# KikeM/romtime

Measured on AMD Instinct MI355X. Metric: snapshot-DoF/s for POD build, higher is better.
Workload: dtype f64

## Files before the change

### include/romtime_hip.h

```cpp
#ifndef ROMTIME_HIP_H
#define ROMTIME_HIP_H

#include <stdint.h>

#ifdef __cplusplus
extern "C" {
#endif

typedef struct rt_ctx rt_ctx;

#define RT_OK 0
#define RT_ERR_ARG (-1)
#define RT_ERR_HIP (-2)
#define RT_ERR_UNSUPPORTED (-3)
#define RT_WARN_ZERO_NORM 1
#define RT_WARN_SINGULAR 2

#define RT_ROW_MAJOR 0
#define RT_COL_MAJOR 1

int rt_version(void);
int rt_ctx_create(rt_ctx** out, int device);
void rt_ctx_destroy(rt_ctx* ctx);
int rt_ctx_set_stream(rt_ctx* ctx, void* hip_stream);
// ... 127 lines not shown
                                      int64_t stride_a, const double* scale, int64_t n_pts, int64_t k, int64_t nt,
                                      int64_t n_traj, int fn, const double* par, const double* out, int64_t* info3);

int rt_interpolation_errors(rt_ctx* ctx, const double* Psi, int64_t ldpsi, const int64_t* idx, int64_t m, const double* F,
                            int64_t ldf, int f_layout, int64_t N, int64_t S, int64_t group, int64_t pin_row, double pin_value,
                            double* err, double* ref);
int rt_interpolation_errors_plan_info(int num_cus, const double* Psi, int64_t ldpsi, const int64_t* idx, int64_t m,
                                      const double* F, int64_t ldf, int f_layout, int64_t N, int64_t S, int64_t group,
                                      int64_t pin_row, double pin_value, const double* err, const double* ref, int64_t* info3);

#define RT_P1_MASS 0
#define RT_P1_STIFFNESS 1
#define RT_P1_CONVECTION 2
#define RT_P1_TRILINEAR 3
#define RT_P1_LOAD 4
#define RT_P1_LOAD_P2 5
int rt_p1_local_assembly(rt_ctx* ctx, int kind, int64_t nx, const int64_t* rows, const int64_t* cols, int64_t m,
                         int64_t n_states, const double* h, const double* coef, int state_mode, const double* state,
                         double* out);

int rt_p1_snapshot_sets(rt_ctx* ctx, int kind, int64_t nx, const int64_t* rows, const int64_t* cols, int64_t m,
                        int64_t n_par, const double* h, const double* coef, int par_mode, const double* par,
                        int64_t n_fun, const double* fun, int zero_first, double beta, double* out);
int rt_p1_snapshot_sets_plan_info(int num_cus, int kind, int64_t nx, const int64_t* rows, const int64_t* cols, int64_t m,
                                  int64_t n_par, const double* h, const double* coef, int par_mode, const double* par,
                                  int64_t n_fun, const double* fun, int zero_first, double beta, const double* out,
                                  int64_t* info2);

typedef struct {
  int64_t nx, n_mu, nt;
  int64_t first_step;
  double dt;
  int bdf2;
  int state_in_w;
  const double* tab;
  const double* u_init;
} rt_fom_desc;
int rt_p1_fom_bdf_sweep(rt_ctx* ctx, const rt_fom_desc* desc, double* U_out, int64_t ld_step, int64_t stride_mu, int* info);
int rt_p1_fom_bdf_sweep_plan_info(int num_cus, const rt_fom_desc* desc, int64_t ld_step, int64_t stride_mu, int64_t* info3);
int rt_p1_fom_bdf_sweep_certified(rt_ctx* ctx, const rt_fom_desc* desc, double* U_out, int64_t ld_step, int64_t stride_mu,
                                  double defect_tol, double* defect, int* info);
int rt_p1_fom_bdf_sweep_certified_plan_info(int num_cus, const rt_fom_desc* desc, int64_t ld_step, int64_t stride_mu,
                                            int64_t* info4);

int rt_trajectory_residuals(rt_ctx* ctx, const rt_fom_desc* desc, const double* B, int64_t ldb, int64_t k, const double* A,
                            int64_t lda, int64_t stride_a, const double* a_init, double* res, double* scale);
int rt_trajectory_residuals_plan_info(int num_cus, const rt_fom_desc* desc, const double* B, int64_t ldb, int64_t k,
                                      const double* A, int64_t lda, int64_t stride_a, const double* a_init, const double* res,
                                      const double* scale, int64_t* info3);

int rt_sym_eig_values(rt_ctx* ctx, const double* G, int64_t n, double* lam, int* status);
int rt_sym_eig_values_part(rt_ctx* ctx, const double* G, int64_t n, int64_t first, int64_t count, double* lam,
                           int* status);
int rt_sym_eig_vectors(rt_ctx* ctx, int64_t n, int64_t k, const double* lam, double* W);

int rt_sym_jacobi_eigh(rt_ctx* ctx, const double* A, int64_t n, double* lam, double* W, int max_sweeps, int* sweeps_done,
                       int* status);

int rt_sym_eig_blocked_plan_info(int64_t n, int64_t block_max, int64_t* p_out, int64_t* widths);
#define RT_EIG_BLOCKED_OK 0
#define RT_EIG_BLOCKED_NOT_REDUCIBLE 1
#define RT_EIG_BLOCKED_SOLVE_FAILED 2
int rt_sym_eig_blocked(rt_ctx* ctx, const double* G, int64_t n, double floor_rel, int64_t k, double* lam, double* W,
                       int64_t* resolved, int64_t* block_ranks, int* status);

int rt_host_jacobi_eigh(double* A, int64_t n, double* W, double* lam, int max_sweeps, int* sweeps_done);

int rt_bench_mfma_f64(rt_ctx* ctx, int iters, double* tflops);
int rt_bench_copy(rt_ctx* ctx, void* dst, const void* src, int64_t bytes, int reps, double* gbps);

#ifdef __cplusplus
}
#endif
#endif
```

### romtime_amd/_lib.py

```python
from __future__ import annotations

import ctypes as C
import os
import threading
import weakref

_HERE = os.path.dirname(os.path.abspath(__file__))
LIB_PATH = os.path.join(_HERE, "lib", "libromtime_hip.so")

ROW_MAJOR, COL_MAJOR = 0, 1
RT_OK = 0
WARN_ZERO_NORM, WARN_SINGULAR = 1, 2
EIG_BLOCKED_OK, EIG_BLOCKED_NOT_REDUCIBLE, EIG_BLOCKED_SOLVE_FAILED = 0, 1, 2

_p = C.c_void_p
_i64 = C.c_int64
_int = C.c_int

SOLVER_DIRECT, SOLVER_GMRES = 0, 1


class GmresOpts(C.Structure):

    _fields_ = [("rtol", C.c_double), ("atol", C.c_double), ("restart", _i64), ("maxiter", _i64)]
# ... 7 lines not shown
    "rt_ctx_synchronize": (_int, [_p]),
    "rt_last_error": (C.c_char_p, [_p]),
    "rt_last_launch_info": (_int, [_p, C.POINTER(_i64)]),
    "rt_ctx_set_profile": (_int, [_p, _int]),
    "rt_ctx_set_option": (_int, [_p, C.c_char_p, _int]),
    "rt_last_gemm_ms": (_int, [_p, C.POINTER(C.c_double)]),
    "rt_last_gram_ms": (_int, [_p, C.POINTER(C.c_double)]),
    "rt_gram_plan_info": (_int, [_int, _i64, _i64, C.POINTER(_int)]),
    "rt_gram_spare_plan_info": (_int, [_int, _i64, _i64, _int, _int, C.POINTER(_int)]),
    "rt_ctx_get_counter": (_int, [_p, C.c_char_p, C.POINTER(_i64)]),
    "rt_stream_create_cu_range": (_int, [_int, _int, _int, C.POINTER(_p)]),
    "rt_stream_destroy": (_int, [_p]),
    "rt_last_sweep_stats": (_int, [_p, C.POINTER(_i64)]),
    "rt_gram": (_int, [_p, _p, _i64, _i64, _i64, _int, _p]),
    "rt_gram_scale": (_int, [_p, _p, _i64, _p, _int, _p]),
    "rt_pod_backproject_weights": (_int, [_p, _p, _i64, _i64, _p, _p, _p]),
    "rt_pod_enqueue": (_int, [_p, _p, _i64, _i64, _i64, _int, _i64, _int, _p, _p, _p, _p, _p, _p, _p]),
    "rt_pod_orth": (_int, [_p, _p, _i64, _i64, _i64, _int, _i64, C.c_double, _int, _p, _i64, C.POINTER(_i64), _p, _p,
                           C.POINTER(_int)]),
    "rt_gemm_tn": (_int, [_p, _p, _i64, _int, _p, _i64, _int, _i64, _i64, _i64, _p, _i64]),
    "rt_gemm_nn": (_int, [_p, _p, _i64, _int, _p, _i64, _i64, _i64, _i64, _p, _i64, _int]),
    "rt_rank_update": (_int, [_p, _p, _i64, _p, _p, _i64, _p, _i64, _i64, _i64, _i64, C.c_double, _p, _i64]),
    "rt_gemm_nn_axpby": (_int, [_p, _p, _i64, _int, _p, _i64, _i64, _i64, _i64, C.c_double, C.c_double, _p, _i64, _int]),
    "rt_transpose": (_int, [_p, _p, _i64, _i64, _i64, _p, _i64]),
    "rt_deim_greedy": (_int, [_p, _p, _i64, _i64, _i64, _int, _p, _p, _p]),
    "rt_csr_spmm": (_int, [_p, _p, _p, _p, _i64, _p, _i64, _i64, _p, _i64]),
    "rt_project_csr": (_int, [_p, _p, _p, _p, _i64, _p, _i64, _i64, _p]),
    "rt_project_csr_batched": (_int, [_p, _p, _p, _p, _i64, _int, _i64, _i64, _p, _i64, _i64, _p]),
    "rt_project_stage_info": (_int, [_p, _p, _p, _i64, C.POINTER(_i64), C.POINTER(_int)]),
    "rt_dense_solve_batched": (_int, [_p, _p, _p, _i64, _i64, _p]),
    "rt_dense_solve_multi": (_int, [_p, _p, _i64, _p, _p, _i64, _p]),
    "rt_tracked_solve_batched": (_int, [_p, _p, _p, _p, _i64, _i64, _int, _p]),
    "rt_gmres_batched": (_int, [_p, _p, _p, _p, _i64, _i64, C.POINTER(GmresOpts), _p, _p]),
    "rt_ctx_set_reduced_solver": (_int, [_p, _int, C.POINTER(GmresOpts)]),
    "rt_rom_bdf_sweep": (_int, [_p, _p, _p]),
    "rt_hrom_bdf_sweep": (_int, [_p, _p, _p]),
    "rt_trajectory_errors": (_int, [_p, _p, _i64, _p, _i64, _i64, _p, _i64, _int, _i64, _i64, _i64, _i64, _i64, _p, _p]),
    "rt_trajectory_integrals": (_int, [_p, _p, _i64, _p, _p, _i64, _i64, _p, _i64, _i64, _i64, _i64, _int, C.POINTER(C.c_double), _p]),
    "rt_trajectory_integrals_plan_info": (_int, [_int, _p, _i64, _p, _p, _i64, _i64, _p, _i64, _i64, _i64, _i64, _int,
                                                 C.POINTER(C.c_double), _p, C.POINTER(_i64)]),
    "rt_interpolation_errors": (_int, [_p, _p, _i64, C.POINTER(_i64), _i64, _p, _i64, _int, _i64, _i64, _i64, _i64, C.c_double, _p, _p]),
    "rt_interpolation_errors_plan_info": (_int, [_int, _p, _i64, C.POINTER(_i64), _i64, _p, _i64, _int, _i64, _i64, _i64, _i64,
                                                 C.c_double, _p, _p, C.POINTER(_i64)]),
    "rt_p1_local_assembly": (_int, [_p, _int, _i64, _p, _p, _i64, _i64, _p, _p, _int, _p, _p]),
    "rt_p1_snapshot_sets": (_int, [_p, _int, _i64, _p, _p, _i64, _i64, _p, _p, _int, _p, _i64, _p, _int, C.c_double, _p]),
    "rt_p1_snapshot_sets_plan_info": (_int, [_int, _int, _i64, _p, _p, _i64, _i64, _p, _p, _int, _p, _i64, _p, _int, C.c_double, _p,
                                             C.POINTER(_i64)]),
    "rt_p1_fom_bdf_sweep": (_int, [_p, _p, _p, _i64, _i64, _p]),
    "rt_p1_fom_bdf_sweep_plan_info": (_int, [_int, _p, _i64, _i64, C.POINTER(_i64)]),
    "rt_p1_fom_bdf_sweep_certified": (_int, [_p, _p, _p, _i64, _i64, C.c_double, _p, _p]),
    "rt_p1_fom_bdf_sweep_certified_plan_info": (_int, [_int, _p, _i64, _i64, C.POINTER(_i64)]),
    "rt_trajectory_residuals": (_int, [_p, _p, _p, _i64, _i64, _p, _i64, _i64, _p, _p, _p]),
    "rt_trajectory_residuals_plan_info": (_int, [_int, _p, _p, _i64, _i64, _p, _i64, _i64, _p, _p, _p, C.POINTER(_i64)]),
    "rt_sym_eig_values": (_int, [_p, _p, _i64, _p, _p]),
    "rt_sym_eig_values_part": (_int, [_p, _p, _i64, _i64, _i64, _p, _p]),
    "rt_sym_eig_vectors": (_int, [_p, _i64, _i64, _p, _p]),
    "rt_sym_eig_blocked_plan_info": (_int, [_i64, _i64, C.POINTER(_i64), C.POINTER(_i64)]),
    "rt_sym_eig_blocked": (_int, [_p, _p, _i64, C.c_double, _i64, _p, _p, C.POINTER(_i64), C.POINTER(_i64), C.POINTER(_int)]),
    "rt_sym_jacobi_eigh": (_int, [_p, _p, _i64, _p, _p, _int, C.POINTER(_int), _p]),
    "rt_host_jacobi_eigh": (_int, [_p, _i64, _p, _p, _int, C.POINTER(_int)]),
    "rt_bench_mfma_f64": (_int, [_p, _int, C.POINTER(C.c_double)]),
    "rt_bench_copy": (_int, [_p, _p, _p, _i64, _int, C.POINTER(C.c_double)]),
}



class SweepDesc(C.Structure):

    _fields_ = [("N", _i64), ("nnz", _i64), ("r", _i64), ("n_mu", _i64), ("nt", _i64), ("dt", C.c_double),
                ("bdf2", _int), ("indptr", _p), ("indices", _p), ("V", _p), ("mass_values", _p), ("n_terms", _i64),
                ("term_values", _p), ("term_coef", _p), ("tril_values", _p), ("n_rhs", _i64), ("rhs_terms", _p),
                ("rhs_coef", _p)]


class HSweepDesc(C.Structure):

    _fields_ = [("r", _i64), ("n_mu", _i64), ("nt", _i64), ("dt", C.c_double), ("bdf2", _int), ("m_mass", _i64),
                ("m_lin", _i64), ("m_nl", _i64), ("m_rhs", _i64), ("Z", _p), ("Zf", _p), ("F_mass", _p), ("F_lin", _p),
                ("F_rhs", _p), ("W", _p), ("C_nl", _p), ("S_nl", _p)]


class FomDesc(C.Structure):

    _fields_ = [("nx", _i64), ("n_mu", _i64), ("nt", _i64), ("first_step", _i64), ("dt", C.c_double), ("bdf2", _int),
                ("state_in_w", _int), ("tab", _p), ("u_init", _p)]


_lib = None
_lock = threading.Lock()


class RomtimeHipError(RuntimeError):
    pass


def load():
    global _lib
    with _lock:
        if _lib is not None:
            return _lib
        if not os.path.exists(LIB_PATH):
            raise RomtimeHipError(
                f"{LIB_PATH} is missing: build it with `python -m romtime_amd.build` "
                "(hipcc --offload-arch=gfx950). romtime_amd has no CPU fallback."
            )
        lib = C.CDLL(LIB_PATH)
# ... 146 lines not shown
```

### romtime_amd/csrc/api.hip

```cpp
#include "common.h"

#include <chrono>
#include <new>

namespace {

int grow(rt_ctx* ctx, void** buf, size_t* have, size_t bytes, void** out) {
  if (bytes > *have) {
    RT_HIP_CHECK(ctx, hipStreamSynchronize(ctx->stream));
    if (*buf) RT_HIP_CHECK(ctx, hipFree(*buf));
    *buf = nullptr;
    *have = 0;
    const size_t want = (bytes + ((size_t)1 << 20) - 1) & ~(((size_t)1 << 20) - 1);
    RT_HIP_CHECK(ctx, hipMalloc(buf, want));
    *have = want;
  }
  *out = *buf;
  return RT_OK;
}

__global__ void gram_scale_kernel(double* __restrict__ G, int n, double* __restrict__ colnorm, int normalize,
                                  int* status_flag) {
  const long idx = (long)blockIdx.x * blockDim.x + threadIdx.x;
  if (idx >= (long)n * n) return;
// ... 103 lines not shown
      s += a;
    }
  }
  if (s == -1.2345) sink[0] = s;
}

__global__ __launch_bounds__(256) void copy_kernel(double4* __restrict__ dst, const double4* __restrict__ src, long n4) {
  const long stride = (long)gridDim.x * blockDim.x;
  for (long i = (long)blockIdx.x * blockDim.x + threadIdx.x; i < n4; i += stride) dst[i] = src[i];
}

}

int rt_scratch(rt_ctx* ctx, size_t bytes, void** out) { return grow(ctx, &ctx->scratch, &ctx->scratch_bytes, bytes, out); }
int rt_scratch2(rt_ctx* ctx, size_t bytes, void** out) {
  ++ctx->scratch2_gen;
  return grow(ctx, &ctx->scratch2, &ctx->scratch2_bytes, bytes, out);
}

int rt_func_lds(rt_ctx* ctx, const void* fn, int bytes) {
  for (const void* f : ctx->lds_done)
    if (f == fn) return RT_OK;
  RT_HIP_CHECK(ctx, hipFuncSetAttribute(fn, hipFuncAttributeMaxDynamicSharedMemorySize, bytes));
  ctx->lds_done.push_back(fn);
  return RT_OK;
}

int rt_profile_begin(rt_ctx* ctx, bool also_gram) {
  if (!ctx->profile) return RT_OK;
  if (!ctx->ev0) {
    RT_HIP_CHECK(ctx, hipEventCreate(&ctx->ev0));
    RT_HIP_CHECK(ctx, hipEventCreate(&ctx->ev1));
  }
  if (also_gram && !ctx->gev0) {
    RT_HIP_CHECK(ctx, hipEventCreate(&ctx->gev0));
    RT_HIP_CHECK(ctx, hipEventCreate(&ctx->gev1));
  }
  RT_HIP_CHECK(ctx, hipEventRecord(ctx->ev0, ctx->stream));
  if (also_gram) RT_HIP_CHECK(ctx, hipEventRecord(ctx->gev0, ctx->stream));
  return RT_OK;
}

int rt_profile_end(rt_ctx* ctx, bool also_gram) {
  if (!ctx->profile) return RT_OK;
  RT_HIP_CHECK(ctx, hipEventRecord(ctx->ev1, ctx->stream));
  if (also_gram) RT_HIP_CHECK(ctx, hipEventRecord(ctx->gev1, ctx->stream));
  ctx->ev_valid = true;
  if (also_gram) ctx->gev_valid = true;
  return RT_OK;
}

extern "C" {

int rt_version(void) { return 440; }

int rt_ctx_create(rt_ctx** out, int device) {
  if (!out) return RT_ERR_ARG;
  *out = nullptr;
  int count = 0;
  if (hipGetDeviceCount(&count) != hipSuccess || device < 0 || device >= count) return RT_ERR_HIP;
  if (hipSetDevice(device) != hipSuccess) return RT_ERR_HIP;
  rt_ctx* ctx = new (std::nothrow) rt_ctx();
  if (!ctx) return RT_ERR_HIP;
  ctx->device = device;
  hipDeviceProp_t prop;
  if (hipGetDeviceProperties(&prop, device) == hipSuccess) ctx->num_cus = ctx->device_cus = prop.multiProcessorCount;
  if (hipMalloc(reinterpret_cast<void**>(&ctx->dev_counters), sizeof(long) * RT_N_COUNTERS) != hipSuccess ||
      hipMemset(ctx->dev_counters, 0, sizeof(long) * RT_N_COUNTERS) != hipSuccess) {
    delete ctx;
    return RT_ERR_HIP;
  }
  *out = ctx;
  return RT_OK;
}

void rt_ctx_destroy(rt_ctx* ctx) {
  if (!ctx) return;
  (void)hipSetDevice(ctx->device);
  (void)hipDeviceSynchronize();
  if (ctx->scratch) (void)hipFree(ctx->scratch);
  if (ctx->scratch2) (void)hipFree(ctx->scratch2);
  if (ctx->dev_counters) (void)hipFree(ctx->dev_counters);
  if (ctx->gram_pace) (void)hipFree(ctx->gram_pace);
  if (ctx->ev0) (void)hipEventDestroy(ctx->ev0);
  if (ctx->ev1) (void)hipEventDestroy(ctx->ev1);
  if (ctx->gev0) (void)hipEventDestroy(ctx->gev0);
  if (ctx->gev1) (void)hipEventDestroy(ctx->gev1);
  delete ctx;
}

int rt_ctx_set_stream(rt_ctx* ctx, void* hip_stream) {
  if (!ctx) return RT_ERR_ARG;
  ctx->stream = static_cast<hipStream_t>(hip_stream);
  return RT_OK;
}

int rt_stream_create_cu_range(int device, int first_cu_per_xcd, int n_cu_per_xcd, void** stream) {
  if (!stream) return RT_ERR_ARG;
  *stream = nullptr;
  hipDeviceProp_t prop;
  if (hipSetDevice(device) != hipSuccess || hipGetDeviceProperties(&prop, device) != hipSuccess) return RT_ERR_HIP;
  const int per_xcd = prop.multiProcessorCount / 8;
  if (first_cu_per_xcd < 0 || n_cu_per_xcd < 1 || first_cu_per_xcd + n_cu_per_xcd > per_xcd) return RT_ERR_ARG;
  const int words = (prop.multiProcessorCount + 31) / 32;
  std::vector<uint32_t> mask((size_t)words, 0u);
  for (int cu = first_cu_per_xcd; cu < first_cu_per_xcd + n_cu_per_xcd; ++cu)
    for (int xcd = 0; xcd < 8; ++xcd) {
      const int bit = cu * 8 + xcd;
      mask[bit >> 5] |= 1u << (bit & 31);
    }
  hipStream_t st = nullptr;
  if (hipExtStreamCreateWithCUMask(&st, (uint32_t)words, mask.data()) != hipSuccess) return RT_ERR_HIP;
  *stream = st;
  return RT_OK;
}

int rt_stream_destroy(void* stream) {
  if (!stream) return RT_ERR_ARG;
  return hipStreamDestroy(static_cast<hipStream_t>(stream)) == hipSuccess ? RT_OK : RT_ERR_HIP;
}

int rt_ctx_synchronize(rt_ctx* ctx) {
  if (!ctx) return RT_ERR_ARG;
  RT_HIP_CHECK(ctx, hipStreamSynchronize(ctx->stream));
  return RT_OK;
}

const char* rt_last_error(rt_ctx* ctx) { return ctx ? ctx->err.c_str() : "null ctx"; }

int rt_last_launch_info(rt_ctx* ctx, int64_t* info3) {
  if (!ctx || !info3) return RT_ERR_ARG;
  info3[0] = ctx->last_grid;
  info3[1] = ctx->last_splits;
  info3[2] = ctx->last_tile;
  return RT_OK;
}

int rt_ctx_set_option(rt_ctx* ctx, const char* name, int value) {
  if (!ctx || !name) return RT_ERR_ARG;
  const std::string key(name);
  if (key == "eig_one_xcd") {
    ctx->eig_one_xcd = value != 0;
    return RT_OK;
  }
  if (key == "eig_xcd") {
    if (value < 0 || value > 7) {
      ctx->err = "rt_ctx_set_option: eig_xcd must be 0 .. 7";
      return RT_ERR_ARG;
    }
    ctx->eig_xcd = value;
    return RT_OK;
  }
  if (key == "gram_pace") {
    ctx->gram_pace_on = value != 0;
    return RT_OK;
  }
  if (key == "pod_blocked") {
    ctx->pod_blocked = value != 0;
    return RT_OK;
  }
  if (key == "sweep_graph") {
    ctx->sweep_graph = value != 0;
    return RT_OK;
  }
  if (key == "cu_limit") {
    if (value < 0 || value > ctx->device_cus || (value % 8) != 0) {
      ctx->err = "rt_ctx_set_option: cu_limit must be a multiple of 8 between 0 and the device's CU count";
      return RT_ERR_ARG;
    }
    ctx->num_cus = value ? value : ctx->device_cus;
    return RT_OK;
  }
  ctx->err = "rt_ctx_set_option: unknown option " + key;
  return RT_ERR_ARG;
}

int rt_ctx_get_counter(rt_ctx* ctx, const char* name, int64_t* value) {
  if (!ctx || !name || !value) return RT_ERR_ARG;
  const std::string key(name);
  static const struct { const char* name; int slot; } table[] = {
      {"eig_timeouts", RT_CNT_EIG_TIMEOUT}, {"eig_general_form", RT_CNT_EIG_GENERAL_FORM},
      {"eig_one_xcd", RT_CNT_EIG_ONE_XCD}, {"gram_off_xcd", RT_CNT_GRAM_OFF_XCD}, {"sweep_newton_iterations", RT_CNT_NS_ITER},
      {"sweep_restarts", RT_CNT_NS_RESTART}, {"sweep_lu_fallbacks", RT_CNT_LU_FALLBACK}, {"sweep_solves", RT_CNT_SOLVES},
      {"sweep_gmres_iterations", RT_CNT_GMRES_ITER}, {"sweep_gmres_unconverged", RT_CNT_GMRES_UNCONVERGED},
      {"eig_wide_form", RT_CNT_EIG_WIDE_FORM}, {"eig_blocked", RT_CNT_EIG_BLOCKED},
      {"eig_blocked_not_reducible", RT_CNT_EIG_BLOCKED_NOT_REDUCIBLE}, {"eig_blocked_rank", RT_CNT_EIG_BLOCKED_RANK}};
  for (const auto& t : table)
    if (key == t.name) {
      long host = 0;
      RT_HIP_CHECK(ctx, hipMemcpyAsync(&host, ctx->dev_counters + t.slot, sizeof(long), hipMemcpyDeviceToHost, ctx->stream));
      RT_HIP_CHECK(ctx, hipStreamSynchronize(ctx->stream));
      *value = host;
      return RT_OK;
    }
  ctx->err = "rt_ctx_get_counter: unknown counter " + key;
  return RT_ERR_ARG;
}

int rt_last_sweep_stats(rt_ctx* ctx, int64_t* stats4) {
  if (!ctx || !stats4) return RT_ERR_ARG;
  long host[4];
  RT_HIP_CHECK(ctx, hipMemcpyAsync(host, ctx->dev_counters + RT_CNT_NS_ITER, sizeof(host), hipMemcpyDeviceToHost, ctx->stream));
  RT_HIP_CHECK(ctx, hipStreamSynchronize(ctx->stream));
// ... 181 lines not shown
```

### romtime_amd/csrc/common.h

```cpp
#pragma once
#include <hip/hip_runtime.h>
#include <stdint.h>
#include <string>
#include <vector>

#include "../../include/romtime_hip.h"

typedef double d2 __attribute__((ext_vector_type(2)));
typedef double d4 __attribute__((ext_vector_type(4)));

constexpr int RT_N_COUNTERS = 14;

struct rt_ctx {
  int device = 0;
  hipStream_t stream = nullptr;
  void* scratch = nullptr;
  size_t scratch_bytes = 0;
  void* scratch2 = nullptr;
  size_t scratch2_bytes = 0;
  int num_cus = 256;
  int device_cus = 256;
  std::string err;
  int64_t last_grid = 0, last_splits = 0, last_tile = 0;
  bool profile = false;
  hipEvent_t ev0 = nullptr, ev1 = nullptr;
  bool ev_valid = false;
  hipEvent_t gev0 = nullptr, gev1 = nullptr;
  bool gev_valid = false;
  bool sweep_graph = false;
  bool eig_one_xcd = true;
  int eig_xcd = 0;
  struct {
    const double *d = nullptr, *e = nullptr, *V = nullptr, *tau = nullptr;
    int64_t n = 0;
    void* base = nullptr;
    uint64_t gen = 0;
  } eig;
  uint64_t scratch2_gen = 0;
  std::vector<const void*> lds_done;
  long* dev_counters = nullptr;
  unsigned long long* gram_pace = nullptr;
  bool gram_pace_on = true;
  bool pod_blocked = false;
  int reduced_solver = RT_SOLVER_DIRECT;
  rt_gmres_opts gmres_opts{1e-5, 0.0, 20, 1};
};

enum {
  RT_CNT_EIG_TIMEOUT = 0,
  RT_CNT_EIG_GENERAL_FORM = 1,
  RT_CNT_EIG_ONE_XCD = 2,
  RT_CNT_GRAM_OFF_XCD = 3,
  RT_CNT_NS_ITER = 4,
  RT_CNT_NS_RESTART = 5,
  RT_CNT_LU_FALLBACK = 6,
  RT_CNT_SOLVES = 7,
  RT_CNT_GMRES_ITER = 8,
  RT_CNT_GMRES_UNCONVERGED = 9,
  RT_CNT_EIG_WIDE_FORM = 10,
  RT_CNT_EIG_BLOCKED = 11,
  RT_CNT_EIG_BLOCKED_NOT_REDUCIBLE = 12,
  RT_CNT_EIG_BLOCKED_RANK = 13
};

#define RT_TRY(expr)                 \
  do {                               \
    const int _rc = (expr);          \
    if (_rc != RT_OK) return _rc;    \
  } while (0)

int rt_func_lds(rt_ctx* ctx, const void* fn, int bytes);

#define RT_HIP_CHECK(ctx, expr)                                                              \
  do {                                                                                       \
    hipError_t _e = (expr);                                                                  \
    if (_e != hipSuccess) {                                                                  \
      (ctx)->err = std::string(#expr) + ": " + hipGetErrorString(_e);                        \
      return RT_ERR_HIP;                                                                     \
    }                                                                                        \
  } while (0)

#define RT_ARG_CHECK(ctx, cond)                                                              \
  do {                                                                                       \
    if (!(cond)) {                                                                           \
// ... 56 lines not shown
```

### romtime_amd/csrc/symeig.hip

```cpp
#include <type_traits>

#include "common.h"
#include "wave_ops.h"

namespace {

constexpr int TW_SMALL = 32;
constexpr int SLOT0 = 160;
constexpr int TW_LARGE = 128;
constexpr int LPR = 64;
constexpr int TT = 1024;
static_assert(LPR == 64, "row reductions use the whole-wave DPP sum");
constexpr int NMAX = 1024;
constexpr int VEC_ITERS = 2;

struct TriParams {
  const double* G;
  double* V;
  double* P;
  double* tau;
  double* d;
  double* e;
  int* flags;
  int n;
// ... 322 lines not shown
  double glo = 1e300, ghi = -1e300, emax = 0.0;
  for (int i = lane; i < n; i += 64) {
    const double di = d[i], ei = (i + 1 < n) ? e[i] : 0.0, el = (i > 0) ? fabs(e[i - 1]) : 0.0;
    sd[i] = di;
    se2[i] = ei * ei;
    glo = fmin(glo, di - el - fabs(ei));
    ghi = fmax(ghi, di + el + fabs(ei));
    emax = fmax(emax, ei * ei);
  }
  glo = rtw::wave_min(glo);
  ghi = rtw::wave_max(ghi);
  emax = rtw::wave_max(emax);
  __syncthreads();
  const double tn = fmax(fabs(glo), fabs(ghi));
  double lo = glo - 2.2e-16 * tn * n - 1e-300, hi = ghi + 2.2e-16 * tn * n + 1e-300;
  const double pivmin = 2.2250738585072014e-308 * fmax(1.0, emax);
  const int j = first + min(2 * (int)blockIdx.x + (wid >> 1), count - 1);
  const int want = n - j;
  constexpr int NSH = 128 * BIS_NS;
  constexpr int NSEC = NSH + 1;
  for (int pass = 0; pass < 7; ++pass) {
    const double h = (hi - lo) / NSEC;
    const int s0 = BIS_NS * (64 * half + lane);
    const double x0 = lo + h * (s0 + 1), x1 = x0 + h;
    double q0 = sd[0] - x0, q1 = sd[0] - x1;
    if (fabs(q0) < pivmin) q0 = -pivmin;
    if (fabs(q1) < pivmin) q1 = -pivmin;
    int c0 = (q0 < 0.0), c1 = (q1 < 0.0);
    for (int i = 1; i < n; ++i) {
      const double di = sd[i], ei = se2[i - 1];
      q0 = fma(-ei, fast_rcp(q0), di - x0);
      q1 = fma(-ei, fast_rcp(q1), di - x1);
      if (fabs(q0) < pivmin) q0 = -pivmin;
      if (fabs(q1) < pivmin) q1 = -pivmin;
      c0 += (q0 < 0.0); c1 += (q1 < 0.0);
    }
    int first = NSH;
    if (c1 >= want) first = s0 + 1;
    if (c0 >= want) first = s0;
    first = rtw::wave_min_i32(first);
    if (lane == 0) s_first[pass & 1][wid] = first;
    __syncthreads();
    first = min(s_first[pass & 1][wid & 2], s_first[pass & 1][(wid & 2) + 1]);
    if (first == NSH) {
      lo = lo + h * NSH;
    } else {
      hi = lo + h * (first + 1);
      lo = lo + h * first;
    }
  }
  if (lane == 0 && half == 0) lam[j] = 0.5 * (lo + hi);
}

struct VecParams {
  const double* d;
  const double* e;
  const double* lam;
  const double* V;
  const double* tau;
  const double* C;
  double* W;
  int n, k;
};

constexpr int RBK = 4;

template <int NM>
__global__ __launch_bounds__(64) void symeig_wy_kernel(const double* __restrict__ V, int n, double* __restrict__ C) {
  constexpr int PER = NM / 64;
  const int b = blockIdx.x, lane = threadIdx.x, k0 = n - 3 - RBK * b;
  double v[RBK][PER];
#pragma unroll
  for (int u = 0; u < RBK; ++u)
#pragma unroll
    for (int q = 0; q < PER; ++q) {
      const int k = k0 - u, j = lane + 64 * q;
      v[u][q] = (k >= 0 && j > k && j < n) ? V[(size_t)k * n + j] : 0.0;
    }
  int slot = 0;
#pragma unroll
  for (int u = 1; u < RBK; ++u)
#pragma unroll
    for (int w = 0; w < u; ++w) {
      double dot = 0.0;
#pragma unroll
      for (int q = 0; q < PER; ++q) dot = fma(v[u][q], v[w][q], dot);
      dot = rtw::wave_sum(dot);
      if (lane == 0) C[6 * b + slot] = dot;
      ++slot;
    }
}

template <int NM>
__global__ __launch_bounds__(64) void symeig_vectors_kernel(const VecParams p) {
  extern __shared__ __attribute__((aligned(16))) double vsm[];
  double *dd = vsm, *ee = dd + NM, *ra = ee + NM + 8, *ub = ra + NM, *ud = ub + NM, *lm = ud + NM, *z = lm + NM,
         *y = z + NM;
  unsigned char* piv = reinterpret_cast<unsigned char*>(y + NM);
  const int n = p.n, t = blockIdx.x, lane = threadIdx.x;
  const double lambda = p.lam[t];
  double tnorm = 0.0;
  for (int i = lane; i < n; i += 64) {
    dd[i] = p.d[i] - lambda;
    ee[i] = (i + 1 < n) ? p.e[i] : 0.0;
    tnorm = fmax(tnorm, fabs(p.d[i]) + 2.0 * ((i + 1 < n) ? fabs(p.e[i]) : 0.0));
    unsigned s = 1664525u * (unsigned)(i + 1 + 7919 * (t + 1)) + 1013904223u;
// ... 265 lines not shown
      const int j = tid + WIDE_T * q;
      const double vq = (j == kk + 1) ? 1.0 : ((j > kk + 1 && j < n) ? x[q] * scale : 0.0);
      if (j < lda) vn[j] = vq;
      if (j > kk && j < n) p.V[(size_t)kk * n + j] = vq;
    }
    if (tid == 0) {
      p.tau[kk] = tk;
      p.d[kk] = diag;
      p.e[kk] = beta;
    }
  } else {
    if (tid == 0) {
      p.d[kk] = diag;
      p.e[kk] = alpha;
      p.e[n - 1] = 0.0;
    }
#pragma unroll
    for (int q = 0; q < PER; ++q)
      if (tid + WIDE_T * q == n - 1) {
#pragma clang fp contract(off)
        p.d[n - 1] = p.A[(size_t)(n - 1) * lda + (n - 1)] - (v[q] * w[q] + w[q] * v[q]);
      }
  }
}
static_assert(NWIDE % WIDE_CHUNK == 0 && NWIDE % WIDE_T == 0, "the reflector kernel covers a padded row with PER elements per thread");

template <int LO, int HI, class F>
int size_class(int64_t n, F&& f) {
  if constexpr (LO < HI)
    if (n > LO) return size_class<2 * LO, HI>(n, f);
  return f(std::integral_constant<int, LO>{});
}

struct EigArena {
  void* base;
  double *V, *own, *tau, *d, *e;
  int* flags;
  int carve(rt_ctx* ctx, int64_t n, size_t own_bytes) {
    rt_carver a;
    const size_t oV = a.add(sizeof(double) * n * n), oO = a.add(own_bytes), oT = a.add(sizeof(double) * n),
                 oD = a.add(sizeof(double) * n), oE = a.add(sizeof(double) * n), oF = a.add(sizeof(int) * (SLOT0 + TW_LARGE));
    RT_TRY(rt_scratch2(ctx, a.total(), &base));
    V = a.at<double>(base, oV); own = a.at<double>(base, oO);
    tau = a.at<double>(base, oT); d = a.at<double>(base, oD);
    e = a.at<double>(base, oE); flags = a.at<int>(base, oF);
    return RT_OK;
  }
  void publish(rt_ctx* ctx, int64_t n) const {
    ctx->eig.d = d; ctx->eig.e = e; ctx->eig.V = V; ctx->eig.tau = tau; ctx->eig.n = n; ctx->eig.base = base;
    ctx->eig.gen = ctx->scratch2_gen;
  }
};

int launch_bisect(rt_ctx* ctx, const EigArena& a, int64_t n, int64_t first, int64_t count, double* lam, int* status) {
  return size_class<512, NWIDE>(n, [&](auto nm) {
    hipLaunchKernelGGL(symeig_bisect_kernel<decltype(nm)::value>, dim3((unsigned)((count + 1) / 2)), dim3(256), 0, ctx->stream, a.d,
                       a.e, (int)n, (int)first, (int)count, lam, a.flags, status, ctx->dev_counters);
    RT_HIP_CHECK(ctx, hipGetLastError());
    return (int)RT_OK;
  });
}

}

static int sym_eig_values_wide(rt_ctx* ctx, const double* G, int64_t n, int64_t first, int64_t count, double* lam,
                               int* status) {
  const int lda = (int)((n + WIDE_CHUNK - 1) / WIDE_CHUNK * WIDE_CHUNK);
  const size_t nvec = (size_t)3 * (lda + WIDE_ROWS) + (size_t)(n + WIDE_ROWS);
  static_assert(sizeof(double) * WIDE_CHUNK % 256 == 0, "the vector buffers start on a 256-byte boundary");
  const size_t cells = (size_t)(n + WIDE_ROWS) * lda;
  EigArena ar;
  RT_TRY(ar.carve(ctx, n, sizeof(double) * (cells + nvec)));
  WideParams wp;
  wp.V = ar.V; wp.A = ar.own;
  wp.vb = wp.A + cells; wp.w = wp.vb + (size_t)2 * (lda + WIDE_ROWS);
  wp.pr = wp.w + (lda + WIDE_ROWS);
  wp.tau = ar.tau; wp.d = ar.d; wp.e = ar.e;
  wp.n = (int)n; wp.lda = lda; wp.counters = ctx->dev_counters;
  hipStream_t st = ctx->stream;
  hipLaunchKernelGGL(symeig_init_kernel, dim3(1), dim3(256), 0, st, ar.flags, wp.tau, (int)n);
  hipLaunchKernelGGL(symeig_wide_load_kernel, dim3((unsigned)((cells + WIDE_T - 1) / WIDE_T)), dim3(WIDE_T), 0, st, G, wp,
                     (long)nvec);
  hipLaunchKernelGGL(symeig_wide_reflect_kernel, dim3(1), dim3(WIDE_T), 0, st, wp, -1);
  RT_HIP_CHECK(ctx, hipGetLastError());
  for (int k = 0; k + 2 < (int)n; ++k) {
    const int rows = (int)n - 1 - k;
    hipLaunchKernelGGL(symeig_wide_sweep_kernel, dim3((unsigned)((rows + WIDE_ROWS - 1) / WIDE_ROWS)), dim3(WIDE_T), 0, st, wp, k);
    hipLaunchKernelGGL(symeig_wide_reflect_kernel, dim3(1), dim3(WIDE_T), 0, st, wp, k);
  }
  RT_HIP_CHECK(ctx, hipGetLastError());
  RT_TRY(launch_bisect(ctx, ar, n, first, count, lam, status));
  ar.publish(ctx, n);
  return RT_OK;
}

extern "C" int rt_sym_eig_values(rt_ctx* ctx, const double* G, int64_t n, double* lam, int* status) {
  return rt_sym_eig_values_part(ctx, G, n, 0, n, lam, status);
}

extern "C" int rt_sym_eig_values_part(rt_ctx* ctx, const double* G, int64_t n, int64_t first, int64_t count, double* lam,
                                      int* status) {
  if (!ctx) return RT_ERR_ARG;
  RT_ARG_CHECK(ctx, G && lam && n >= 3 && first >= 0 && count >= 1 && first + count <= n);
  if (n > NWIDE) {
    ctx->err = "rt_sym_eig_values: n > 2048 not supported (the limit of the device eigensolver)";
    return RT_ERR_UNSUPPORTED;
  }
  if (n > NMAX) return sym_eig_values_wide(ctx, G, n, first, count, lam, status);
  const bool large = n > 512;
  const bool small_team = !large && ctx->num_cus < TW_SMALL && ctx->num_cus >= TW_SMALL / 2;
  int tw = large ? TW_LARGE : (small_team ? TW_SMALL / 2 : TW_SMALL);
  const bool local = n <= 64;
  if (local) tw = 1;
  if (tw > ctx->num_cus) {
    ctx->err = "rt_sym_eig_values: not enough compute units for the cooperative tridiagonalisation";
    return RT_ERR_UNSUPPORTED;
  }
  EigArena ar;
  RT_TRY(ar.carve(ctx, n, sizeof(double) * 4 * n));
  TriParams tp;
  tp.G = G; tp.n = (int)n; tp.tw = tw;
  tp.spread = (!large && !local && ctx->eig_one_xcd && ctx->num_cus / 8 >= tw) ? 1 : 0;
  tp.local = local ? 1 : 0;
  tp.xcd = ctx->eig_xcd & 7;
  tp.V = ar.V; tp.P = ar.own; tp.tau = ar.tau; tp.d = ar.d; tp.e = ar.e; tp.flags = ar.flags;
  tp.counters = ctx->dev_counters;
  hipStream_t st = ctx->stream;
  hipLaunchKernelGGL(symeig_init_kernel, dim3(1), dim3(256), 0, st, tp.flags, tp.tau, (int)n);

  const int RB = (int)((n + tw - 1) / tw);
  const size_t lds = sizeof(double) * ((size_t)RB * (local ? n + 2 : n) + 5 * n + 16);
  const auto tridiag = [&](auto nm) -> int {
    const auto kernel = &symeig_tridiag_kernel<decltype(nm)::value>;
    RT_TRY(rt_func_lds(ctx, reinterpret_cast<const void*>(kernel), 150 * 1024));
    int per_cu = 0;
    RT_HIP_CHECK(ctx, hipOccupancyMaxActiveBlocksPerMultiprocessor(&per_cu, kernel, TT, lds));
    if ((long)per_cu * ctx->num_cus < tw) {
      ctx->err = "rt_sym_eig_values: the device cannot keep all cooperating workgroups resident";
      return RT_ERR_UNSUPPORTED;
    }
    hipLaunchKernelGGL(kernel, dim3(tp.spread ? 16 * tw : tw), dim3(TT), lds, st, tp);
    RT_HIP_CHECK(ctx, hipGetLastError());
    return RT_OK;
  };
  RT_TRY((size_class<128, NMAX>(n, tridiag)));
  RT_TRY(launch_bisect(ctx, ar, n, first, count, lam, status));
  ar.publish(ctx, n);
  return RT_OK;
// ... 30 lines not shown
```

### romtime_amd/csrc/wave_ops.h

```cpp
#pragma once
#include <hip/hip_runtime.h>

namespace rtw {

template <int CTRL, int ROW_MASK = 0xf, int BANK_MASK = 0xf>
__device__ __forceinline__ double dpp_f64(double x) {
  const long long b = __double_as_longlong(x);
  int lo = (int)b, hi = (int)(b >> 32);
  lo = __builtin_amdgcn_update_dpp(0, lo, CTRL, ROW_MASK, BANK_MASK, false);
  hi = __builtin_amdgcn_update_dpp(0, hi, CTRL, ROW_MASK, BANK_MASK, false);
  return __longlong_as_double(((long long)hi << 32) | (unsigned)lo);
}

__device__ __forceinline__ double read_lane(double x, int lane) {
  const long long b = __double_as_longlong(x);
  const int lo = __builtin_amdgcn_readlane((int)b, lane), hi = __builtin_amdgcn_readlane((int)(b >> 32), lane);
  return __longlong_as_double(((long long)hi << 32) | (unsigned)lo);
}

__device__ __forceinline__ double first_lane(double x) {
  const long long b = __double_as_longlong(x);
  const int lo = __builtin_amdgcn_readfirstlane((int)b), hi = __builtin_amdgcn_readfirstlane((int)(b >> 32));
  return __longlong_as_double(((long long)hi << 32) | (unsigned)lo);
}

__device__ __forceinline__ double wave_sum(double x) {
  x += dpp_f64<0xb1>(x);
  x += dpp_f64<0x4e>(x);
  x += dpp_f64<0x114>(x);
  x += dpp_f64<0x118>(x);
  x += dpp_f64<0x142, 0xa>(x);
  x += dpp_f64<0x143, 0xc>(x);
  return read_lane(x, 63);
}

template <int CTRL, int ROW_MASK = 0xf, int BANK_MASK = 0xf>
__device__ __forceinline__ int dpp_keep_i32(int x) {
  return __builtin_amdgcn_update_dpp(x, x, CTRL, ROW_MASK, BANK_MASK, false);
}
template <int CTRL, int ROW_MASK = 0xf, int BANK_MASK = 0xf>
__device__ __forceinline__ double dpp_keep_f64(double x) {
  const long long b = __double_as_longlong(x);
  const int lo = dpp_keep_i32<CTRL, ROW_MASK, BANK_MASK>((int)b), hi = dpp_keep_i32<CTRL, ROW_MASK, BANK_MASK>((int)(b >> 32));
  return __longlong_as_double(((long long)hi << 32) | (unsigned)lo);
}

__device__ __forceinline__ double wave_max(double x) {
  x = fmax(x, dpp_keep_f64<0xb1>(x));
  x = fmax(x, dpp_keep_f64<0x4e>(x));
  x = fmax(x, dpp_keep_f64<0x114>(x));
  x = fmax(x, dpp_keep_f64<0x118>(x));
  x = fmax(x, dpp_keep_f64<0x142, 0xa>(x));
  x = fmax(x, dpp_keep_f64<0x143, 0xc>(x));
  return read_lane(x, 63);
}

__device__ __forceinline__ double wave_min(double x) {
  x = fmin(x, dpp_keep_f64<0xb1>(x));
  x = fmin(x, dpp_keep_f64<0x4e>(x));
  x = fmin(x, dpp_keep_f64<0x114>(x));
  x = fmin(x, dpp_keep_f64<0x118>(x));
  x = fmin(x, dpp_keep_f64<0x142, 0xa>(x));
  x = fmin(x, dpp_keep_f64<0x143, 0xc>(x));
  return read_lane(x, 63);
}

__device__ __forceinline__ int wave_min_i32(int x) {
  x = min(x, dpp_keep_i32<0xb1>(x));
  x = min(x, dpp_keep_i32<0x4e>(x));
  x = min(x, dpp_keep_i32<0x114>(x));
  x = min(x, dpp_keep_i32<0x118>(x));
  x = min(x, dpp_keep_i32<0x142, 0xa>(x));
  x = min(x, dpp_keep_i32<0x143, 0xc>(x));
  return __builtin_amdgcn_readlane(x, 63);
}

template <int CTRL, int ROW_MASK = 0xf, int BANK_MASK = 0xf>
__device__ __forceinline__ void argmax_step(double& v, int& i) {
  const double ov = dpp_keep_f64<CTRL, ROW_MASK, BANK_MASK>(v);
  const int oi = dpp_keep_i32<CTRL, ROW_MASK, BANK_MASK>(i);
  const bool take = ov > v || (ov == v && oi < i);
  v = take ? ov : v;
  i = take ? oi : i;
}
__device__ __forceinline__ void wave_argmax(double& v, int& i) {
  argmax_step<0xb1>(v, i);
  argmax_step<0x4e>(v, i);
  argmax_step<0x114>(v, i);
  argmax_step<0x118>(v, i);
  argmax_step<0x142, 0xa>(v, i);
  argmax_step<0x143, 0xc>(v, i);
  v = read_lane(v, 63);
  i = __builtin_amdgcn_readlane(i, 63);
}

}
```

### romtime_amd/pipeline.py

```python
from __future__ import annotations

import collections
import ctypes as C
import os
import weakref

import torch

from . import _lib, ops, pod, pod_rules

_p = C.c_void_p


SMALL_SET = 150_000_000
_STREAMS: dict = {}
_STREAMS_PID: list = []
_OPEN_RUNS = weakref.WeakSet()


def shutdown():
    import gc

    if not _STREAMS:
        return
# ... 16 lines not shown

def _masked_stream(lib, dev, first, count):
    key = (dev, first, count)
    if key not in _STREAMS:
        h = _p()
        rc = lib.rt_stream_create_cu_range(dev, first, count, C.byref(h))
        if rc != 0:
            raise _lib.RomtimeHipError(f"rt_stream_create_cu_range({first}, {count}) failed ({rc})")
        _STREAMS[key] = torch.cuda.ExternalStream(h.value, device=torch.device("cuda", dev))
        _STREAMS_PID[:] = [os.getpid()]
    return _STREAMS[key]


import atexit

atexit.register(shutdown)


def _checked(X, runner):
    if X.dim() != 2 or not X.is_cuda or X.dtype != torch.float64:
        raise _lib.RomtimeHipError(f"{type(runner).__name__} takes 2-D float64 CUDA tensors")
    return X


def _wait_for(waiters, stream):
    ev = torch.cuda.Event()
    ev.record(stream)
    for st in waiters:
        st.wait_event(ev)


class PodPipeline:
    def __init__(self, eig_cus_per_xcd: int = 4, device=None, group=None, eig_first_cu: int = 0, gram_range=None,
                 small_set=None, gram_pace: bool = False):
        self.small_set = SMALL_SET if small_set is None else int(small_set)
        if not torch.cuda.is_available():
            raise _lib.RomtimeHipError("no MI355X visible: romtime_amd's hot path runs on the GPU only")
        self.device = torch.device("cuda", torch.cuda.current_device() if device is None else device)
        dev = self.device.index
        lib = _lib.load()
        self.lib = lib
        per_xcd = torch.cuda.get_device_properties(dev).multi_processor_count // 8
        e = int(eig_cus_per_xcd)
        if not (1 <= e < per_xcd):
            raise ValueError(f"eig_cus_per_xcd must be in [1, {per_xcd})")
        g_first, g_count = gram_range if gram_range is not None else (eig_first_cu + e, per_xcd - e - eig_first_cu)
        if eig_first_cu < 0 or g_count < 1 or g_first + g_count > per_xcd or not (eig_first_cu + e <= g_first or g_first + g_count <= eig_first_cu):
            raise ValueError("the CU ranges of the two streams must be disjoint and inside the XCD")
        self.sE = _masked_stream(lib, dev, eig_first_cu, e)
        self.sG = _masked_stream(lib, dev, g_first, g_count)
        self.ctxE, self.ctxG = _lib.Context(dev), _lib.Context(dev)
        self.ctxE.set_option("cu_limit", 8 * e)
        self.ctxE.set_option("eig_one_xcd", 0)
        self.ctxG.set_option("cu_limit", 8 * g_count)
        self.ctxG.set_option("gram_pace", int(bool(gram_pace)))
        self.group = group
        self.group_e, self.world, self.rank = None, 1, 0
        if group is not None:
            import torch.distributed as dist

            if dist.get_world_size(group) > 1 or os.environ.get("ROMTIME_FORCE_COLLECTIVES"):
                self.group_e = dist.new_group(ranks=dist.get_process_group_ranks(group), backend=dist.get_backend(group))
                self.world, self.rank = dist.get_world_size(group), dist.get_rank(group)
        self.sC = torch.cuda.Stream(self.device) if self.group_e is not None else None
        self.sR = self.sE if self.group_e is not None else None
        self.eig_cus = 8 * e
        self.recomputed = 0
        self.gram_kernel_ms = []
        self.last_stage_ms = {}

    def close(self):
        torch.cuda.synchronize(self.device)

    def _gram(self, item):
        X = item["X"]
        n = X.shape[1]
        with self.ctxG.use(self.sG):
            item["t0"] = torch.cuda.Event(enable_timing=True)
            item["t0"].record()
            Gbuf = torch.empty(n * n + 1, dtype=torch.float64, device=X.device)
            item["G"] = ops.gram(X, out=Gbuf[: n * n].view(n, n))
            Gbuf[n * n:].fill_(float(X.shape[0]))
            item["k0"] = torch.cuda.Event(enable_timing=True)
            item["k0"].record()
            item["Gbuf"] = Gbuf
        st = self.sG if self.sR is None else self.sR
        with torch.cuda.stream(st):
            if st is not self.sG:
                st.wait_event(item["k0"])
            if self.group is not None:
                import torch.distributed as dist

                dist.all_reduce(Gbuf, op=dist.ReduceOp.SUM, group=self.group)
            item["g"] = torch.cuda.Event(enable_timing=True)
            item["g"].record()

    def _eig(self, item):
        k, normalize = item["k"], item["normalize"]
        item["owner"] = item["index"] % self.world
        if self.rank != item["owner"]:
            return
        with self.ctxE.use(self.sE):
            self.sE.wait_event(item["g"])
            G = item["G"]
            n = G.shape[0]
            colnorm, flag = ops.gram_scale(G, normalize)
# ... 300 lines not shown
```

Before: 93.76 billion.

## Add shared-wave multisection eigenvalue bisection kernel for small CU budgets

Adds a bisection kernel where each eigenvalue is computed by a group of S lanes (8, 16 or 32) evaluating Sturm counts at S shifts per pass, instead of a whole workgroup per pair of eigenvalues. A planner chooses between the whole-workgroup plan and the shared plans from CU count, matrix size and pass count, requiring all workgroups to be resident at once. The pipeline's eig context, which is limited to a few CUs, enables this mode. The intent is to cut the tail of the eigenvalue stage when there are more eigenvalues than CUs, at the cost of more multisection passes per eigenvalue.

After: 94.04 billion, median of 4. About the same (+0.3%).

```diff
diff --git a/include/romtime_hip.h b/include/romtime_hip.h
--- a/include/romtime_hip.h
+++ b/include/romtime_hip.h
@@ -203,6 +203,7 @@
 int rt_sym_eig_values(rt_ctx* ctx, const double* G, int64_t n, double* lam, int* status);
 int rt_sym_eig_values_part(rt_ctx* ctx, const double* G, int64_t n, int64_t first, int64_t count, double* lam,
                            int* status);
+int rt_bisect_plan_info(int num_cus, int64_t n, int64_t count, int* out);
 int rt_sym_eig_vectors(rt_ctx* ctx, int64_t n, int64_t k, const double* lam, double* W);
 
 int rt_sym_jacobi_eigh(rt_ctx* ctx, const double* A, int64_t n, double* lam, double* W, int max_sweeps, int* sweeps_done,
diff --git a/romtime_amd/_lib.py b/romtime_amd/_lib.py
--- a/romtime_amd/_lib.py
+++ b/romtime_amd/_lib.py
@@ -83,6 +83,7 @@
     "rt_p1_fom_bdf_sweep_certified_plan_info": (_int, [_int, _p, _i64, _i64, C.POINTER(_i64)]),
     "rt_trajectory_residuals": (_int, [_p, _p, _p, _i64, _i64, _p, _i64, _i64, _p, _p, _p]),
     "rt_trajectory_residuals_plan_info": (_int, [_int, _p, _p, _i64, _i64, _p, _i64, _i64, _p, _p, _p, C.POINTER(_i64)]),
+    "rt_bisect_plan_info": (_int, [_int, _i64, _i64, C.POINTER(_int)]),
     "rt_sym_eig_values": (_int, [_p, _p, _i64, _p, _p]),
     "rt_sym_eig_values_part": (_int, [_p, _p, _i64, _i64, _i64, _p, _p]),
     "rt_sym_eig_vectors": (_int, [_p, _i64, _i64, _p, _p]),
diff --git a/romtime_amd/csrc/api.hip b/romtime_amd/csrc/api.hip
--- a/romtime_amd/csrc/api.hip
+++ b/romtime_amd/csrc/api.hip
@@ -179,7 +179,7 @@
 
 extern "C" {
 
-int rt_version(void) { return 440; }
+int rt_version(void) { return 450; }
 
 int rt_ctx_create(rt_ctx** out, int device) {
   if (!out) return RT_ERR_ARG;
@@ -276,6 +276,14 @@
       return RT_ERR_ARG;
     }
     ctx->eig_xcd = value;
+    return RT_OK;
+  }
+  if (key == "eig_bisect_share") {
+    if (value != 0 && value != 1 && value != 8 && value != 16 && value != 32) {
+      ctx->err = "rt_ctx_set_option: eig_bisect_share must be 0, 1, 8, 16 or 32";
+      return RT_ERR_ARG;
+    }
+    ctx->eig_bisect_share = value;
     return RT_OK;
   }
   if (key == "gram_pace") {
diff --git a/romtime_amd/csrc/common.h b/romtime_amd/csrc/common.h
--- a/romtime_amd/csrc/common.h
+++ b/romtime_amd/csrc/common.h
@@ -30,6 +30,7 @@
   bool sweep_graph = false;
   bool eig_one_xcd = true;
   int eig_xcd = 0;
+  int eig_bisect_share = 0;
   struct {
     const double *d = nullptr, *e = nullptr, *V = nullptr, *tau = nullptr;
     int64_t n = 0;
diff --git a/romtime_amd/csrc/symeig.hip b/romtime_amd/csrc/symeig.hip
--- a/romtime_amd/csrc/symeig.hip
+++ b/romtime_amd/csrc/symeig.hip
@@ -398,6 +398,76 @@
   if (lane == 0 && half == 0) lam[j] = 0.5 * (lo + hi);
 }
 
+constexpr int BIS_SHARE_WAVES = 8;
+constexpr int bis_passes(int S) {
+  constexpr unsigned long long target = 257ull * 257 * 257 * 257 * 257 * 257 * 257;
+  unsigned long long v = 1;
+  int p = 0;
+  while (v < target) {
+    v *= (unsigned long long)(S + 1);
+    ++p;
+  }
+  return p;
+}
+static_assert(bis_passes(256) == 7 && bis_passes(32) == 12 && bis_passes(16) == 14 && bis_passes(8) == 18, "");
+
+template <int NM, int S>
+__global__ __launch_bounds__(256, BIS_SHARE_WAVES) void symeig_bisect_share_kernel(
+    const double* __restrict__ d, const double* __restrict__ e, int n, int first, int count, double* __restrict__ lam,
+    const int* flags, int* status, long* counters) {
+  if (blockIdx.x == 0 && threadIdx.x == 0) {
+    if (status) *status = flags[3];
+    if (flags[3]) atomicAdd(reinterpret_cast<unsigned long long*>(&counters[RT_CNT_EIG_TIMEOUT]), 1ull);
+  }
+  __shared__ double sd[NM], se2[NM];
+  constexpr int EPW = 64 / S;
+  const int tid = threadIdx.x, lane = tid & 63, wid = tid >> 6, grp = lane / S, sl = lane % S;
+  double glo = 1e300, ghi = -1e300, emax = 0.0;
+  for (int i = lane; i < n; i += 64) {
+    const double di = d[i], ei = (i + 1 < n) ? e[i] : 0.0, el = (i > 0) ? fabs(e[i - 1]) : 0.0;
+    sd[i] = di;
+    se2[i] = ei * ei;
+    glo = fmin(glo, di - el - fabs(ei));
+    ghi = fmax(ghi, di + el + fabs(ei));
+    emax = fmax(emax, ei * ei);
+  }
+  glo = rtw::wave_min(glo);
+  ghi = rtw::wave_max(ghi);
+  emax = rtw::wave_max(emax);
+  __syncthreads();
+  const double tn = fmax(fabs(glo), fabs(ghi));
+  double lo = glo - 2.2e-16 * tn * n - 1e-300, hi = ghi + 2.2e-16 * tn * n + 1e-300;
+  const double pivmin = 2.2250738585072014e-308 * fmax(1.0, emax);
+  const int j = first + min((4 * (int)blockIdx.x + wid) * EPW + grp, count - 1);
+  const int want = n - j;
+  constexpr int NSH = S;
+  constexpr int NSEC = NSH + 1;
+  for (int pass = 0; pass < bis_passes(S); ++pass) {
+    const double h = (hi - lo) / NSEC;
+    const int s0 = sl;
+    const double x0 = lo + h * (s0 + 1);
+    double q0 = sd[0] - x0;
+    if (fabs(q0) < pivmin) q0 = -pivmin;
+    int c0 = (q0 < 0.0);
+    for (int i = 1; i < n; ++i) {
+      const double di = sd[i], ei = se2[i - 1];
+      q0 = fma(-ei, fast_rcp(q0), di - x0);
+      if (fabs(q0) < pivmin) q0 = -pivmin;
+      c0 += (q0 < 0.0);
+    }
+    int first = NSH;
+    if (c0 >= want) first = s0;
+    first = rtw::group_min_i32<S>(first);
+    if (first == NSH) {
+      lo = lo + h * NSH;
+    } else {
+      hi = lo + h * (first + 1);
+      lo = lo + h * first;
+    }
+  }
+  if (sl == 0) lam[j] = 0.5 * (lo + hi);
+}
+
 struct VecParams {
   const double* d;
   const double* e;
@@ -769,7 +839,59 @@
   }
 };
 
+struct BisectPlan {
+  int shifts, passes, lanes, workgroups;
+};
+constexpr int BIS_SHARE_NMAX = 512;
+BisectPlan bisect_whole_plan(long count) { return {128 * BIS_NS, 7, 128, (int)((count + 1) / 2)}; }
+BisectPlan bisect_share_plan(int S, long count) {
+  const long per_wg = 4 * (64 / S);
+  return {S, bis_passes(S), S, (int)((count + per_wg - 1) / per_wg)};
+}
+bool bisect_share_resident(const BisectPlan& p, int num_cus) { return (long)p.workgroups <= (long)num_cus * BIS_SHARE_WAVES; }
+BisectPlan bisect_choose(int num_cus, long n, long count, int forced = 0) {
+  const BisectPlan whole = bisect_whole_plan(count);
+  if (n > BIS_SHARE_NMAX) return whole;
+  if (forced) return bisect_share_plan(forced, count);
+  if (whole.workgroups <= num_cus) return whole;
+  BisectPlan best = {};
+  double best_t = 0.0;
+  for (int S : {32, 16, 8}) {
+    const BisectPlan p = bisect_share_plan(S, count);
+    if (!bisect_share_resident(p, num_cus)) continue;
+    const double deep = (double)p.workgroups / num_cus;
+    const double t = (deep > 1.0 ? deep : 1.0) * p.passes;
+    if (best.shifts == 0 || t < best_t) {
+      best = p;
+      best_t = t;
+    }
+  }
+  return best.shifts ? best : whole;
+}
+
 int launch_bisect(rt_ctx* ctx, const EigArena& a, int64_t n, int64_t first, int64_t count, double* lam, int* status) {
+  const int opt = ctx->eig_bisect_share;
+  const BisectPlan plan = opt == 0 ? bisect_whole_plan((long)count) : bisect_choose(ctx->num_cus, (long)n, (long)count, opt > 1 ? opt : 0);
+  if (plan.shifts != 128 * BIS_NS) {
+    if (!bisect_share_resident(plan, ctx->num_cus)) {
+      ctx->err = "rt_sym_eig_values: the multisection's workgroups would not be resident at once on this ctx's CUs";
+      return RT_ERR_UNSUPPORTED;
+    }
+    const auto share = [&](auto nm, auto s) {
+      hipLaunchKernelGGL((symeig_bisect_share_kernel<decltype(nm)::value, decltype(s)::value>), dim3((unsigned)plan.workgroups),
+                         dim3(256), 0, ctx->stream, a.d, a.e, (int)n, (int)first, (int)count, lam, a.flags, status,
+                         ctx->dev_counters);
+      RT_HIP_CHECK(ctx, hipGetLastError());
+      return (int)RT_OK;
+    };
+    return size_class<128, BIS_SHARE_NMAX>(n, [&](auto nm) {
+      switch (plan.shifts) {
+        case 8: return share(nm, std::integral_constant<int, 8>{});
+        case 16: return share(nm, std::integral_constant<int, 16>{});
+        default: return share(nm, std::integral_constant<int, 32>{});
+      }
+    });
+  }
   return size_class<512, NWIDE>(n, [&](auto nm) {
     hipLaunchKernelGGL(symeig_bisect_kernel<decltype(nm)::value>, dim3((unsigned)((count + 1) / 2)), dim3(256), 0, ctx->stream, a.d,
                        a.e, (int)n, (int)first, (int)count, lam, a.flags, status, ctx->dev_counters);
@@ -811,6 +933,13 @@
   return RT_OK;
 }
 
+extern "C" int rt_bisect_plan_info(int num_cus, int64_t n, int64_t count, int* out) {
+  if (!out || num_cus < 8 || n < 3 || n > NWIDE || count < 1 || count > n) return RT_ERR_ARG;
+  const BisectPlan p = bisect_choose(num_cus, (long)n, (long)count);
+  out[0] = p.shifts; out[1] = p.passes; out[2] = p.lanes; out[3] = p.workgroups;
+  return RT_OK;
+}
+
 extern "C" int rt_sym_eig_values(rt_ctx* ctx, const double* G, int64_t n, double* lam, int* status) {
   return rt_sym_eig_values_part(ctx, G, n, 0, n, lam, status);
 }
diff --git a/romtime_amd/csrc/wave_ops.h b/romtime_amd/csrc/wave_ops.h
--- a/romtime_amd/csrc/wave_ops.h
+++ b/romtime_amd/csrc/wave_ops.h
@@ -75,6 +75,18 @@
   return __builtin_amdgcn_readlane(x, 63);
 }
 
+template <int G>
+__device__ __forceinline__ int group_min_i32(int x) {
+  static_assert(G == 4 || G == 8 || G == 16 || G == 32 || G == 64, "a power of two from 4 to 64");
+  x = min(x, dpp_keep_i32<0xb1>(x));
+  x = min(x, dpp_keep_i32<0x4e>(x));
+  if constexpr (G >= 8) x = min(x, dpp_keep_i32<0x141>(x));
+  if constexpr (G >= 16) x = min(x, dpp_keep_i32<0x140>(x));
+  if constexpr (G >= 32) x = min(x, __shfl_xor(x, 16));
+  if constexpr (G >= 64) x = min(x, __shfl_xor(x, 32));
+  return x;
+}
+
 template <int CTRL, int ROW_MASK = 0xf, int BANK_MASK = 0xf>
 __device__ __forceinline__ void argmax_step(double& v, int& i) {
   const double ov = dpp_keep_f64<CTRL, ROW_MASK, BANK_MASK>(v);
diff --git a/romtime_amd/pipeline.py b/romtime_amd/pipeline.py
--- a/romtime_amd/pipeline.py
+++ b/romtime_amd/pipeline.py
@@ -92,6 +92,7 @@
         self.ctxE, self.ctxG = _lib.Context(dev), _lib.Context(dev)
         self.ctxE.set_option("cu_limit", 8 * e)
         self.ctxE.set_option("eig_one_xcd", 0)
+        self.ctxE.set_option("eig_bisect_share", 1)
         self.ctxG.set_option("cu_limit", 8 * g_count)
         self.ctxG.set_option("gram_pace", int(bool(gram_pace)))
         self.group = group
```
